# unilight/jatts

Hardware: AMD Instinct MI355X
Metric: audio samples/sec (22.05 kHz) + RTF, FastSpeech2+HiFi-GAN (higher is better)
Workload: dtype f32 (emulated: 3 exact bf16 terms per operand, 7 MFMA products, f32 accumulate; attention / norms / duration predictor exact f32); 1 GPU; FastSpeech2(JSUT conformer 4+4, adim 384)+HiFi-GAN v1 22k, 64 utts x 128 phonemes x 6 frames per GPU; hop=256, parallelism=dp1 (utterance sharding, int16 PCM all-gather)

## Files before the change

### include/jatts_hip.h

```cpp
#ifndef JATTS_HIP_H_
#define JATTS_HIP_H_

#include <stdint.h>

#ifdef __cplusplus
extern "C" {
#endif

#define JATTS_ABI_VERSION 7

#define JATTS_F32 0
#define JATTS_F16 1
#define JATTS_F32S 2
#define JATTS_F32E 3
#define JATTS_F32E6 4

#define JATTS_ACT_NONE 0
#define JATTS_ACT_RELU 1
#define JATTS_ACT_TANH 2
#define JATTS_ACT_SWISH 3
#define JATTS_ACT_MISH 4
#define JATTS_ACT_SNAKEBETA 5

#define JATTS_PAD_ZERO 0
// ... 64 lines not shown
int jatts_conv1d(const jatts_conv_desc* d, void* stream);

int64_t jatts_conv_weight_index(int32_t n, int32_t tap, int32_t c, int32_t n_pad, int32_t c_in);

typedef struct jatts_resunit_desc {
  jatts_ragged rg;
  int32_t dtype;
  int32_t channels;
  int32_t k_w;
  int32_t dil;
  float slope;
  const void* x;
  void* y;
  const void* w1;
  const float* b1;
  const void* w2;
  const float* b2;
  const void* add0;
  const void* add1;
  float out_scale;
  const float* ws1;
  const float* ws2;
  int32_t w_layout;
  int32_t variant;
} jatts_resunit_desc;

int jatts_hifigan_resunit(const jatts_resunit_desc* d, void* stream);

int jatts_resunit_variant(const jatts_resunit_desc* d);

int jatts_resunit_single_conv(int32_t dtype, int32_t w_layout);

int64_t jatts_unit_weight_index_k32(int32_t n, int32_t tap, int32_t c, int32_t channels);

typedef struct jatts_resblock_desc {
  jatts_ragged rg;
  int32_t dtype;
  int32_t channels;
  int32_t k_w;
  int32_t n_units;
  int32_t dil[3];
  float slope;
  const void* x;
  void* y;
  const void* w1[3];
  const float* b1[3];
  const void* w2[3];
  const float* b2[3];
  const void* add0;
  const void* add1;
  float out_scale;
  const float* ws1[3];
  const float* ws2[3];
} jatts_resblock_desc;

int jatts_hifigan_resblock(const jatts_resblock_desc* d, void* stream);

int jatts_masked_loss(const jatts_ragged* rg, const float* a, int32_t lda, const float* b, int32_t ldb, int32_t dim,
                      const int32_t* valid_len, int32_t kind, float log_offset, double scale, float* out, double* workspace,
                      void* stream);
int jatts_conv1d_wgrad(const jatts_ragged* rg, const float* x, int32_t ldx, const float* dy, int32_t ldy, int32_t c_in,
                       int32_t n_out, int32_t k_w, int32_t dil, int32_t pad, float* dw, float* db, float* workspace, void* stream);
int jatts_pack_conv_weight(const float* w, int32_t n_out, int32_t c_in, int32_t k_w, int32_t c_mult, int32_t mode, int32_t dtype,
                           void* out, void* stream);
int jatts_pack_conv_weight_split(const float* w, int32_t n_out, int32_t c_in, int32_t k_w, int32_t c_mult, int32_t mode, void* out, float* inv,
                                 void* stream);
int jatts_pack_conv_weight_bf16x3(const float* w, int32_t n_out, int32_t c_in, int32_t k_w, int32_t c_mult, int32_t dgrad, void* out, void* stream);
int jatts_conv1d_wgrad_emul(const jatts_ragged* rg, const float* x, int32_t ldx, const float* dy, int32_t ldy, int32_t c_in, int32_t n_out, int32_t k_w,
                            int32_t dil, int32_t pad, int32_t dtype, float* dw, float* db, float* workspace, void* stream);
int jatts_col_sum(const float* x, int32_t ld, int64_t rows, int32_t dim, float* out, void* stream);

int jatts_layernorm_bwd(const float* x, int32_t ldx, const float* dy, int32_t lddy, const float* gamma, int64_t rows, int32_t dim,
                        float eps, float* dx, int32_t lddx, float* dgamma, float* dbeta, void* stream);
int jatts_act_fwd(int32_t mode, const float* x, float* y, int64_t n, void* stream);
int jatts_act_bwd(int32_t mode, const float* x, const float* dy, float* dx, int64_t n, void* stream);
int jatts_glu_fwd(const float* x, float* y, int64_t rows, int32_t dim, void* stream);
int jatts_glu_bwd(const float* x, const float* dy, float* dx, int64_t rows, int32_t dim, void* stream);
int jatts_dwconv(const jatts_ragged* rg, const float* x, const float* w, const float* bias, float* y, int32_t dim, int32_t k_w,
                 int32_t pad, int32_t flip, void* stream);
int jatts_dwconv_wgrad(const jatts_ragged* rg, const float* x, const float* dy, float* dw, int32_t dim, int32_t k_w, int32_t pad,
                       void* stream);
int jatts_col_stats(const float* x, const float* y2, int32_t ld, int64_t rows, int32_t dim, const float* shift, const float* mul,
                    int32_t mode, float* out0, float* out1, void* stream);
int jatts_bn_bwd_apply(const float* x, const float* dy, int64_t rows, int32_t dim, const float* mean, const float* rstd,
                       const float* gamma, const float* s_dy, const float* s_dyx, float* dx, void* stream);
int jatts_index_add_rows(const float* src, int32_t ld, const int64_t* idx, int64_t rows, int32_t dim, float scale, int64_t skip,
                         int64_t n_dst, float* dst, void* stream);
int jatts_lr_segment_sum(const jatts_ragged* rg, const int64_t* cum, const int32_t* cu_out, const float* dy, int32_t dim, float* dhs,
                         void* stream);
int jatts_shift_softmax_fwd(const float* ac, const float* bd, int32_t n_batch, int32_t n_heads, int32_t t_len, const int32_t* lens,
                            float scale, int32_t shift_mode, float* p, void* stream);
int jatts_shift_softmax_bwd(const float* p, const float* dp, int32_t n_batch, int32_t n_heads, int32_t t_len, float scale,
                            int32_t shift_mode, float* ds, float* dbd, void* stream);
int jatts_gate_bwd(const float* x, const float* dy, float* dx, int64_t rows, int32_t dim, void* stream);
int jatts_weight_norm_fwd(const float* v, const float* g, int32_t n_out, int32_t row_len, float* w, float* inv_norm, void* stream);
int jatts_weight_norm_bwd(const float* v, const float* g, const float* inv_norm, const float* dw, int32_t n_out, int32_t row_len,
                          float* dv, float* dg, void* stream);
int jatts_split_add(const float* o, const float* h, const float* skip, int64_t rows, int32_t dim, float* h_out, float* skip_out, void* stream);
int jatts_concat2(const float* a, const float* b, int64_t rows, int32_t dim, float* out, void* stream);
int jatts_outer_rows(const float* v, const float* w, const float* bias, int64_t rows, int32_t dim, int32_t accumulate, float* out,
                     void* stream);
int jatts_col_wsum(const float* x, int32_t ld, const float* v, int64_t rows, int32_t dim, float* out, void* stream);
int jatts_row_dot(const float* x, int32_t ld, const float* w, const float* bias, int64_t rows, int32_t dim, float* y, void* stream);
int jatts_masked_loss_bwd(const jatts_ragged* rg, const float* a, int32_t lda, const float* b, int32_t ldb, int32_t dim,
                          const int32_t* valid_len, int32_t kind, float log_offset, float scale, const float* upstream, float* da,
                          int32_t ldda, void* stream);
// ... 221 lines not shown
```

### jatts_amd/_abi.py

```python
import ctypes as C
import os

_HERE = os.path.dirname(os.path.abspath(__file__))
LIB_PATH = os.environ.get("JATTS_HIP_LIB") or os.path.join(_HERE, "lib", "libjatts_hip.so")

F32, F16, F32S, F32E, F32E6 = 0, 1, 2, 3, 4
ABI_VERSION = 7
ACT_NONE, ACT_RELU, ACT_TANH, ACT_SWISH, ACT_MISH, ACT_SNAKEBETA = 0, 1, 2, 3, 4, 5
PRE_NONE, PRE_LRELU = 0, 1
PAD_ZERO, PAD_REFLECT = 0, 1
STATS_ROWS_PER_GROUP = 1024


class Ragged(C.Structure):
    _fields_ = [("cu_rows", C.c_void_p), ("n_seq", C.c_int32), ("max_len", C.c_int32),
                ("len_mul", C.c_int32), ("total_rows", C.c_int32), ("host_lens", C.c_void_p)]


class ConvDesc(C.Structure):
    _fields_ = [
        ("rg", Ragged), ("dtype", C.c_int32), ("n_in", C.c_int32), ("x", C.c_void_p * 3),
        ("ldx", C.c_int32), ("in_scale", C.c_float), ("pre_act", C.c_int32), ("pre_slope", C.c_float),
        ("w", C.c_void_p), ("c_in", C.c_int32), ("n_out", C.c_int32), ("k_w", C.c_int32),
        ("dil", C.c_int32), ("pad", C.c_int32), ("bias", C.c_void_p), ("act", C.c_int32),
        ("alpha", C.c_float), ("resid", C.c_void_p), ("ldr", C.c_int32), ("y", C.c_void_p),
        ("ldy", C.c_int32), ("y_is_f32", C.c_int32), ("y_transposed", C.c_int32), ("y_seq_col0", C.c_void_p),
        ("pad_mode", C.c_int32), ("variant", C.c_int32), ("w_inv", C.c_void_p), ("act_a", C.c_void_p), ("act_b", C.c_void_p),
        ("n_split", C.c_int32), ("ldy2", C.c_int32), ("y2", C.c_void_p), ("y2_seq_col0", C.c_void_p), ("w_layout", C.c_int32),
        ("tap_group_n", C.c_int32), ("tap_a0", C.c_int32), ("tap_b0", C.c_int32), ("tap_k", C.c_int32),
    ]


class ResUnitDesc(C.Structure):
    _fields_ = [
        ("rg", Ragged), ("dtype", C.c_int32), ("channels", C.c_int32), ("k_w", C.c_int32),
        ("dil", C.c_int32), ("slope", C.c_float), ("x", C.c_void_p), ("y", C.c_void_p),
        ("w1", C.c_void_p), ("b1", C.c_void_p), ("w2", C.c_void_p), ("b2", C.c_void_p),
        ("add0", C.c_void_p), ("add1", C.c_void_p), ("out_scale", C.c_float),
        ("ws1", C.c_void_p), ("ws2", C.c_void_p), ("w_layout", C.c_int32), ("variant", C.c_int32),
    ]


class ResBlockDesc(C.Structure):
    _fields_ = [
        ("rg", Ragged), ("dtype", C.c_int32), ("channels", C.c_int32), ("k_w", C.c_int32), ("n_units", C.c_int32),
        ("dil", C.c_int32 * 3), ("slope", C.c_float), ("x", C.c_void_p), ("y", C.c_void_p),
        ("w1", C.c_void_p * 3), ("b1", C.c_void_p * 3), ("w2", C.c_void_p * 3), ("b2", C.c_void_p * 3),
        ("add0", C.c_void_p), ("add1", C.c_void_p), ("out_scale", C.c_float),
        ("ws1", C.c_void_p * 3), ("ws2", C.c_void_p * 3),
    ]


class RelAttnDesc(C.Structure):
    _fields_ = [
        ("rg", Ragged), ("dtype", C.c_int32), ("n_heads", C.c_int32), ("d_k", C.c_int32),
        ("q", C.c_void_p), ("ldq", C.c_int32), ("k", C.c_void_p), ("ldk", C.c_int32),
        ("vt", C.c_void_p), ("ldvt", C.c_int32), ("g", C.c_void_p), ("ldg", C.c_int32),
        ("ku", C.c_void_p), ("scale", C.c_float), ("out", C.c_void_p), ("ldo", C.c_int32),
        ("rel_mode", C.c_int32), ("rel_center", C.c_int32), ("vt_col0", C.c_void_p), ("kv_len", C.c_void_p),
    ]


COLLATE_MAX_FIELDS = 8


class CollateField(C.Structure):
    _fields_ = [("src", C.c_void_p), ("row_start", C.c_void_p), ("row_len", C.c_void_p), ("dst", C.c_void_p),
                ("elem_bytes", C.c_int32), ("dim", C.c_int32), ("t_max", C.c_int32)]


PROTOTYPES = {
    "jatts_abi_version": (C.c_int, []),
    "jatts_last_error": (C.c_char_p, []),
    "jatts_device_info": (C.c_int, [C.c_char_p, C.c_int]),
    "jatts_conv1d": (C.c_int, [C.POINTER(ConvDesc), C.c_void_p]),
    "jatts_conv_weight_index": (C.c_int64, [C.c_int32] * 5),
    "jatts_hifigan_resunit": (C.c_int, [C.POINTER(ResUnitDesc), C.c_void_p]),
    "jatts_resunit_variant": (C.c_int, [C.POINTER(ResUnitDesc)]),
    "jatts_resunit_single_conv": (C.c_int, [C.c_int32, C.c_int32]),
    "jatts_unit_weight_index_k32": (C.c_int64, [C.c_int32] * 4),
    "jatts_hifigan_resblock": (C.c_int, [C.POINTER(ResBlockDesc), C.c_void_p]),
    "jatts_debug_trace": (C.c_int, [C.c_void_p, C.c_int64]),
    "jatts_mfma_probe": (C.c_int, [C.c_int32, C.c_int32, C.c_void_p, C.c_int64, C.c_int32, C.c_int32, C.c_void_p, C.c_void_p, C.c_void_p]),
    "jatts_mfma_probe_flops": (C.c_double, [C.c_int32, C.c_int32, C.c_int32]),
    "jatts_set_workspace": (C.c_int, [C.c_void_p, C.c_int64]),
    "jatts_pack_conv_weight_split": (C.c_int, [C.c_void_p, C.c_int32, C.c_int32, C.c_int32, C.c_int32, C.c_int32, C.c_void_p, C.c_void_p, C.c_void_p]),
    "jatts_bgemm": (C.c_int, [C.c_void_p, C.c_int64, C.c_int64, C.c_int32, C.c_int32, C.c_void_p, C.c_int64, C.c_int64, C.c_int32, C.c_int32,
                              C.c_void_p, C.c_int64, C.c_int64, C.c_int32, C.c_int32, C.c_int32, C.c_int32, C.c_int32, C.c_int32, C.c_float,
                              C.c_int32, C.c_void_p]),
    "jatts_bgemm_emul": (C.c_int, [C.c_void_p, C.c_int64, C.c_int64, C.c_int32, C.c_int32, C.c_void_p, C.c_int64, C.c_int64, C.c_int32, C.c_int32,
                                   C.c_void_p, C.c_int64, C.c_int64, C.c_int32, C.c_int32, C.c_int32, C.c_int32, C.c_int32, C.c_int32, C.c_float,
                                   C.c_int32, C.c_int32, C.c_void_p]),
    "jatts_pcm16": (C.c_int, [C.c_void_p, C.c_int64, C.c_void_p, C.c_void_p]),
    "jatts_alignment_logp": (C.c_int, [C.POINTER(Ragged), C.c_void_p, C.c_int32, C.c_void_p, C.c_void_p, C.c_int32,
                                       C.c_void_p, C.c_int32, C.c_void_p]),
    "jatts_alignment_logp_bwd": (C.c_int, [C.POINTER(Ragged), C.c_void_p, C.c_int32, C.c_void_p, C.c_void_p, C.c_int32, C.c_void_p, C.c_int32,
                                           C.c_void_p, C.c_int32, C.c_void_p, C.c_void_p, C.c_void_p, C.c_void_p]),
    "jatts_mas_viterbi": (C.c_int, [C.POINTER(Ragged), C.c_void_p, C.c_void_p, C.c_int32, C.c_int32, C.c_void_p,
                                    C.c_void_p, C.c_void_p, C.c_void_p]),
    "jatts_hifigan_output": (C.c_int, [C.POINTER(Ragged), C.c_int32, C.POINTER(C.c_void_p), C.c_int32,
                                       C.c_float, C.c_float, C.c_int32, C.c_int32, C.c_void_p, C.c_float,
                                       C.c_void_p, C.c_void_p]),
# ... 161 lines not shown
```

### jatts_amd/csrc/conv_api.hip

```cpp
#include <stdlib.h>

#include "common.h"

unsigned long long* jatts_g_trace = nullptr;
unsigned jatts_g_trace_cap = 0;

int jatts_conv1d_f16(const jatts_conv_desc& d, hipStream_t s);
int jatts_conv1d_f32(const jatts_conv_desc& d, hipStream_t s);
int jatts_conv1d_split(const jatts_conv_desc& d, hipStream_t s);
int jatts_conv1d_emul(const jatts_conv_desc& d, hipStream_t s);
int jatts_resunit_f16_narrow(const jatts_resunit_desc& d, hipStream_t s);
int jatts_resunit_f16_wide(const jatts_resunit_desc& d, hipStream_t s);
int jatts_resunit_f32(const jatts_resunit_desc& d, hipStream_t s);
int jatts_resunit_split(const jatts_resunit_desc& d, hipStream_t s);
int jatts_resunit_emul(const jatts_resunit_desc& d, hipStream_t s, int* pick);
int jatts_resunit1_f16(const jatts_resunit_desc& d, hipStream_t s);
int jatts_resunit1_f32(const jatts_resunit_desc& d, hipStream_t s);
int jatts_resunit1_emul(const jatts_resunit_desc& d, hipStream_t s);
int jatts_resblock_f16(const jatts_resblock_desc& d, hipStream_t s);
int jatts_resblock_f32(const jatts_resblock_desc& d, hipStream_t s);
int jatts_resblock_split(const jatts_resblock_desc& d, hipStream_t s);
int jatts_resblock_emul(const jatts_resblock_desc& d, hipStream_t s);

extern "C" int jatts_debug_trace(void* buf, int64_t n_workgroups) {
// ... 80 lines not shown
  if (d->dtype != JATTS_F16 && d->dtype != JATTS_F32) return jatts_set_error_msg(JATTS_ERR_UNSUPPORTED, "resunit: unsupported channels/dtype (use jatts_conv1d)");
  return JATTS_OK;
}

extern "C" int jatts_hifigan_resunit(const jatts_resunit_desc* d, void* stream) {
  if (const int rc = resunit_check(d)) return rc;
  hipStream_t s = (hipStream_t)stream;
  if (!d->w2) {
    if (const int rc = resunit1_check(d)) return rc;
    if (d->rg.max_len <= 0) return JATTS_OK;
    if (d->dtype == JATTS_F16) return jatts_resunit1_f16(*d, s);
    if (d->dtype == JATTS_F32) return jatts_resunit1_f32(*d, s);
    return jatts_resunit1_emul(*d, s);
  }
  if (d->rg.max_len <= 0) return JATTS_OK;
  if (d->dtype == JATTS_F16) return d->channels <= 64 ? jatts_resunit_f16_narrow(*d, s) : jatts_resunit_f16_wide(*d, s);
  if (d->dtype == JATTS_F32) return jatts_resunit_f32(*d, s);
  if (d->dtype == JATTS_F32S) {
    if (!d->ws1 || !d->ws2) return jatts_set_error_msg(JATTS_ERR_ARG, "resunit: JATTS_F32S needs ws1 / ws2");
    return jatts_resunit_split(*d, s);
  }
  if (d->dtype == JATTS_F32E || d->dtype == JATTS_F32E6) {
    if (d->w_layout != 0 && d->w_layout != 1) return jatts_set_error_msg(JATTS_ERR_ARG, "resunit: w_layout must be 0 or 1");
    return jatts_resunit_emul(*d, s, nullptr);
  }
  if (d->w_layout != 0) return jatts_set_error_msg(JATTS_ERR_ARG, "resunit: w_layout = 1 goes with JATTS_F32E / JATTS_F32E6 only");
  return jatts_set_error_msg(JATTS_ERR_UNSUPPORTED, "resunit: unsupported channels/dtype (use jatts_conv1d)");
}

extern "C" int jatts_resunit_variant(const jatts_resunit_desc* d) {
  if (const int rc = resunit_check(d)) return rc;
  int form = 1;
  if (!d->w2) {
    const int rc = resunit1_check(d);
    return rc ? rc : 1;
  }
  if (d->rg.max_len > 0 && (d->dtype == JATTS_F32E || d->dtype == JATTS_F32E6)) {
    if (d->w_layout != 0 && d->w_layout != 1) return jatts_set_error_msg(JATTS_ERR_ARG, "resunit: w_layout must be 0 or 1");
    if (const int rc = jatts_resunit_emul(*d, nullptr, &form)) return rc;
  }
  return form;
}

extern "C" int jatts_hifigan_resblock(const jatts_resblock_desc* d, void* stream) {
  if (!d || !d->x || !d->y || !d->rg.cu_rows) return jatts_set_error_msg(JATTS_ERR_ARG, "resblock: null pointer");
  if (d->n_units < 1 || d->n_units > 3) return jatts_set_error_msg(JATTS_ERR_ARG, "resblock: 1..3 units");
  for (int u = 0; u < d->n_units; ++u) {
    if (!d->w1[u] || !d->w2[u] || !d->b1[u] || !d->b2[u]) return jatts_set_error_msg(JATTS_ERR_ARG, "resblock: null weights");
    if (d->dil[u] < 1) return jatts_set_error_msg(JATTS_ERR_ARG, "resblock: dil >= 1 required");
  }
  if (d->x == d->y) return jatts_set_error_msg(JATTS_ERR_ARG, "resblock: y must not alias x");
  if (d->k_w < 1 || !(d->k_w & 1)) return jatts_set_error_msg(JATTS_ERR_ARG, "resblock: odd k_w required");
  if (!(d->slope >= 0.f && d->slope <= 1.f)) return jatts_set_error_msg(JATTS_ERR_ARG, "resblock: LeakyReLU slope must be in [0, 1]");
  if (d->dtype == JATTS_F32S) {
    for (int u = 0; u < d->n_units; ++u)
      if (!d->ws1[u] || !d->ws2[u]) return jatts_set_error_msg(JATTS_ERR_ARG, "resblock: JATTS_F32S needs ws1 / ws2");
    if (d->rg.max_len <= 0) return JATTS_OK;
    return jatts_resblock_split(*d, (hipStream_t)stream);
  }
  if (d->dtype == JATTS_F32E || d->dtype == JATTS_F32E6) {
    if (d->rg.max_len <= 0) return JATTS_OK;
    return jatts_resblock_emul(*d, (hipStream_t)stream);
  }
  if (d->dtype != JATTS_F16 && d->dtype != JATTS_F32) return jatts_set_error_msg(JATTS_ERR_ARG, "resblock: unknown dtype");
  if (d->rg.max_len <= 0) return JATTS_OK;
  return d->dtype == JATTS_F16 ? jatts_resblock_f16(*d, (hipStream_t)stream) : jatts_resblock_f32(*d, (hipStream_t)stream);
}
```

### jatts_amd/csrc/resblock_emul.hip

```cpp
#include "resblock_emul_impl.h"

template <typename T>
static int resblock_emul(const jatts_resblock_desc& d, hipStream_t s) {
  switch (d.channels) {
    case 32:
      return launch_resblock_emul<T, 32, 256, 1, 2, 2, 2>(d, s);
    case 64:
      return launch_resblock_emul<T, 64, 128, 2, 2, 2, 2>(d, s);
  }
  return jatts_set_error_msg(JATTS_ERR_UNSUPPORTED, "resblock (emulated): 32 / 64 channels only (use jatts_hifigan_resunit)");
}

int jatts_resblock_emul(const jatts_resblock_desc& d, hipStream_t s) { return d.dtype == JATTS_F32E6 ? resblock_emul<bf3f>(d, s) : resblock_emul<bf3>(d, s); }
```

### jatts_amd/csrc/resunit_emul16_impl.h

```cpp
#pragma once
#include <type_traits>

#include "resunit_emul_impl.h"

#ifndef JATTS_U16_ROWS
#define JATTS_U16_ROWS 1
#endif
#ifndef JATTS_U16_DIAG
#define JATTS_U16_DIAG 0
#endif

namespace {

struct acc2x4 { f32x4 big, small; };
template <typename T> struct Acc16 { typedef f32x4 type; };
template <> struct Acc16<bf3p<7>> { typedef acc2x4 type; };
__device__ __forceinline__ void acc16_set(f32x4& a, int i, float v) { a[i] = v; }
__device__ __forceinline__ void acc16_set(acc2x4& a, int i, float v) { a.small[i] = v; a.big[i] = 0.f; }
__device__ __forceinline__ void acc16_finish(f32x4&) {}
__device__ __forceinline__ void acc16_finish(acc2x4& a) { a.small = a.big + a.small; }
__device__ __forceinline__ f32x4& acc16_val(f32x4& a) { return a; }
__device__ __forceinline__ f32x4& acc16_val(acc2x4& a) { return a.small; }

template <int P> __device__ __forceinline__ void mma16p(const bf3px8<7>& a, const bf3px8<7>& b, acc2x4& c) {
// ... 357 lines not shown
        for (int e = 0; e < 4; ++e) {
          const float a = acc16_val(acc[f][t])[e] * keep;
          v[e] = fmaxf(a, a * d.slope);
        }
        bf16x4 q0, q1, q2;
        bf3_split4(v, q0, q1, q2);
        char* p = hs + (size_t)(col + off) * pitch + (size_t)(n0 >> 3) * 48 + (size_t)(n0 & 4) * 2;
        *reinterpret_cast<bf16x4*>(p) = q0;
        *reinterpret_cast<bf16x4*>(p + 16) = q1;
        *reinterpret_cast<bf16x4*>(p + 32) = q2;
      }
    }
    JATTS_STAMP(12);
    lds_barrier();
    JATTS_STAMP(4);

    bias_acc(bs + C);
    ws.bind((const T*)d.w2, KC32, NFR16, nf0, lane);
    conv16<T, NF, NT, KC32>(acc, ws, 0, K, 1, hs, pitch, col0, lane, nullptr);
    finish_acc();
    JATTS_STAMP(5);

    __syncthreads();
    if constexpr (SLIDE) {
      for (int u = tid; u < (K - 1) * (C / 8); u += NTHR) {
        const int r = u / (C / 8), cu = u % (C / 8);
        Vec8IO<T>::sts(tl + (size_t)r * pitch_t + (size_t)cu * 48, Vec8IO<T>::lds(hs + (size_t)(nout + r) * pitch + (size_t)cu * 48));
      }
    }
    char* ys = smem;
#pragma unroll
    for (int t = 0; t < NT; ++t) {
      const int col = col0 + t * 16 + (lane & 15);
      if (col >= nvalid) continue;
#pragma unroll
      for (int f = 0; f < NF; ++f) {
        const int n0 = (nf0 + f) * 16 + 4 * g4;
        *reinterpret_cast<f32x4*>(ys + (size_t)col * pitch + (size_t)n0 * 4) = acc16_val(acc[f][t]);
      }
    }
    __syncthreads();
    JATTS_STAMP(6);
    {
      const int vrows = nvalid;
      const int64_t g0 = (seq_row0 + t0) * (int64_t)C;
      constexpr bool keep_small = C <= 64;
      const float* xg = (const float*)d.x;
      float* yg = (float*)d.y;
      if constexpr (RREG) {
        constexpr int UPR = C / 8;
        const int n_out = vrows * UPR;
        const bool has_add1 = d.add0 != nullptr && d.add1 != nullptr;
        f32x8 a0[MAXI], a1[MAXI];
        if (d.add0) {
#pragma unroll
          for (int j = 0; j < MAXI; ++j) {
            const int v = tid + j * NTHR;
            if (v < n_out) {
              a0[j] = Vec8IO<float>::ldg((const float*)d.add0 + g0 + (int64_t)v * 8);
              if (has_add1) a1[j] = Vec8IO<float>::ldg((const float*)d.add1 + g0 + (int64_t)v * 8);
            }
          }
        }
#pragma unroll
        for (int j = 0; j < MAXI; ++j) {
          const int v = tid + j * NTHR;
          if (v >= n_out) continue;
          const int ro = v / UPR, cu = v - ro * UPR;
          f32x8 o = Vec8IO<float>::lds(ys + (size_t)ro * pitch + (size_t)cu * 32);
#pragma unroll
          for (int e = 0; e < 8; ++e) o[e] = o[e] + xk[j][e];
          if (d.add0) {
#pragma unroll
            for (int e = 0; e < 8; ++e) o[e] = (o[e] + a0[j][e] + (has_add1 ? a1[j][e] : 0.f)) * d.out_scale;
          }
          float* dst = yg + g0 + (int64_t)v * 8;
          *reinterpret_cast<f32x4*>(dst) = f32x4{o[0], o[1], o[2], o[3]};
          *reinterpret_cast<f32x4*>(dst + 4) = f32x4{o[4], o[5], o[6], o[7]};
        }
      } else {
        if (d.add0) unit_store_pass<float, C, keep_small ? 2 : 4, true, NTHR>(d.add0, d.add1, d.out_scale, ys, pitch, vrows, xg, yg, g0);
        else unit_store_pass<float, C, keep_small ? 4 : 8, false, NTHR>(d.add0, d.add1, d.out_scale, ys, pitch, vrows, xg, yg, g0);
      }
    }
    JATTS_STAMP(7);
    if constexpr (!SLIDE) break;
    t0 += nout;
    slide = true;
    if (t0 >= L) {
      f_seq += L;
      if (f_seq >= f_end) break;
      do { ++b; } while (d.rg.cu_rows[b + 1] == d.rg.cu_rows[b]);
      t0 = 0;
      slide = false;
    } else if (f_seq + t0 >= f_end) {
      break;
    }
  }
  JATTS_TRACE_END();
}

inline int resunit16_pick(const jatts_resunit_desc& d, int runs, int wgcols, bool slide_auto, bool slide_fits) {
  const int64_t positions = ragged_is_1d(d.rg) ? (int64_t)d.rg.total_rows * d.rg.len_mul : (int64_t)d.rg.n_seq * d.rg.max_len * d.rg.len_mul;
  const bool slide = d.variant == 2 || (d.variant == 0 && slide_auto && positions >= 2 * (int64_t)runs * wgcols);
  return slide && slide_fits ? 2 : 1;
}

template <typename T, int C, int WGCOLS, int WN, int WT, int OCC = 2, bool KSPLIT = false, bool RREG = false>
int launch_resunit_emul16(const jatts_resunit_desc& d, hipStream_t s, int* pick) {
  const int K = d.k_w, p2 = (K - 1) / 2, p1 = p2 * d.dil;
  const int tt_out = WGCOLS - 2 * p2;
  if (tt_out < 8) return jatts_set_error_msg(JATTS_ERR_UNSUPPORTED, "resunit: kernel too wide for tile");
  const size_t pitch = C * 6 + 16, pitch_x = KSPLIT ? (C / 2) * 6 + 16 : pitch;
  const size_t rows_x = WGCOLS + 2 * p1, rows_h = WGCOLS + K - 1;
  if (KSPLIT && 2 * p1 > 64) return jatts_set_error_msg(JATTS_ERR_UNSUPPORTED, "resunit (emulated, channel halves): halo beyond 32 rows a side");
  const size_t region = rows_x * pitch_x > rows_h * pitch ? rows_x * pitch_x : rows_h * pitch;
  const size_t tail = (size_t)(K - 1) * C * 6;
  const size_t lds = region + 2 * C * sizeof(float);
  if (lds > 160 * 1024) return jatts_set_error_msg(JATTS_ERR_UNSUPPORTED, "resunit: tile exceeds 160 KiB LDS");
  int dev = 0, cus = 0;
  hipError_t e = hipGetDevice(&dev);
  if (e == hipSuccess) e = hipDeviceGetAttribute(&cus, hipDeviceAttributeMultiprocessorCount, dev);
  if (e != hipSuccess) return jatts_set_error(e, __FILE__, __LINE__);
  const int runs = cus * OCC;
  const int form = resunit16_pick(d, runs, WGCOLS, !RREG, lds + tail <= 160 * 1024);
  if (pick) {
    *pick = form;
    return JATTS_OK;
  }
  if (form == 2) {
    constexpr auto kern = resunit_emul16_kernel<T, C, WGCOLS, WN, WT, OCC, KSPLIT, RREG, true>;
    if (const int rc = unit_lds_ready<kern>(JATTS_SITE("resunit: tile exceeds 160 KiB LDS"), lds + tail)) return rc;
    hipLaunchKernelGGL(kern, dim3((unsigned)runs), dim3(WN * WT * 64), lds + tail, s, d, jatts_g_trace, jatts_g_trace_cap, (unsigned)(region + tail));
    JATTS_CHECK_LAUNCH();
    return JATTS_OK;
  }
  constexpr auto kern = resunit_emul16_kernel<T, C, WGCOLS, WN, WT, OCC, KSPLIT, RREG>;
  return unit_launch<kern>(JATTS_SITE("resunit: tile exceeds 160 KiB LDS"), WN * WT * 64, lds, tt_out, d.rg, s, d, jatts_g_trace, jatts_g_trace_cap, (unsigned)region);
}

}
```

### jatts_amd/hip.py

```python
import collections
import contextlib
import ctypes as C

import torch

from . import _abi
from . import precision as _precision
from ._abi import ACT_MISH, ACT_NONE, ACT_RELU, ACT_SWISH, ACT_TANH, F16, F32, F32E, F32E6, F32S
from .precision import EMUL, PRECISIONS

_TORCH = {F32: torch.float32, F16: torch.float16, F32S: torch.float32, F32E: torch.float32, F32E6: torch.float32}


def torch_dtype(code):
    return _TORCH[code]


def code_of(t):
    if t.dtype == torch.float32:
        return F32
    if t.dtype == torch.float16:
        return F16
    raise TypeError(f"unsupported dtype {t.dtype}")

# ... 620 lines not shown


def _check_unit_weights(who, dtype, channels, k_w, *ws):
    n = channels * channels * k_w
    want = {F32: (torch.float32, n), F16: (torch.float16, n), F32S: (torch.float16, 2 * n), F32E: (torch.bfloat16, 3 * n), F32E6: (torch.bfloat16, 3 * n)}[dtype]
    for w in ws:
        if w.dtype != want[0] or w.numel() != want[1] or not w.is_cuda:
            raise ValueError(f"{who}: dtype code {dtype} needs packed weights of {want[1]} x {want[0]} on the GPU (pack_conv_weight / pack_conv_weight_split / "
                             f"pack_conv_weight_bf16x3 with c_mult=32), got {w.numel()} x {w.dtype}")


def _resunit_desc(rb, len_mul, x, y, w1, b1, w2, b2, channels, k_w, dil, slope, dtype, add, out_scale, ws, w_layout, variant):
    d = _abi.ResUnitDesc()
    d.w_layout, d.variant = w_layout, variant
    d.rg = rb.struct(len_mul)
    d.dtype, d.channels, d.k_w, d.dil, d.slope = dtype, channels, k_w, dil, slope
    rows = rb.total * len_mul
    if x.numel() != rows * channels or y.numel() != rows * channels or x.dtype != torch_dtype(dtype):
        raise ValueError("hifigan_resunit: bad buffer size/dtype")
    d.x, d.y = _dev(x).data_ptr(), y.data_ptr()
    _check_unit_weights("hifigan_resunit", dtype, channels, k_w, *((w1,) if w2 is None else (w1, w2)))
    d.w1, d.b1, d.w2, d.b2 = w1.data_ptr(), b1.data_ptr(), _ptr(w2), _ptr(b2)
    if dtype == F32S:
        need = ws[:1] if ws is not None and w2 is None else ws
        if need is None or any(v is None or v.numel() < channels or v.dtype != torch.float32 for v in need):
            raise ValueError("hifigan_resunit: F32S needs the inverse weight scales (pack_conv_weight_split)")
        d.ws1, d.ws2 = ws[0].data_ptr(), _ptr(ws[1]) if len(ws) > 1 else None
    if add:
        for a in add:
            if a.numel() != rows * channels or a.dtype != x.dtype:
                raise ValueError("hifigan_resunit: bad mix buffer")
        d.add0 = add[0].data_ptr()
        d.add1 = add[1].data_ptr() if len(add) > 1 else None
    d.out_scale = out_scale
    return d


def hifigan_resunit(rb, len_mul, x, y, w1, b1, w2, b2, channels, k_w, dil, slope, dtype, add=None, out_scale=1.0, ws=None, w_layout=0, variant=0):
    lib = _abi.load()
    d = _resunit_desc(rb, len_mul, x, y, w1, b1, w2, b2, channels, k_w, dil, slope, dtype, add, out_scale, ws, w_layout, variant)
    with _Timed("resunit", (channels, k_w, dil, rb.total * len_mul, len(add) if add else 0)):
        _abi.check(lib.jatts_hifigan_resunit(C.byref(d), _stream()), "jatts_hifigan_resunit")
    return y


def resunit_variant(rb, len_mul, x, y, w1, b1, w2, b2, channels, k_w, dil, slope, dtype, add=None, out_scale=1.0, ws=None, w_layout=0, variant=0):
    lib = _abi.load()
    d = _resunit_desc(rb, len_mul, x, y, w1, b1, w2, b2, channels, k_w, dil, slope, dtype, add, out_scale, ws, w_layout, variant)
    rc = lib.jatts_resunit_variant(C.byref(d))
    _abi.check(min(rc, 0), "jatts_resunit_variant")
    return rc


def hifigan_resblock(rb, len_mul, x, y, units, channels, k_w, slope, dtype, add=None, out_scale=1.0, ws=None):
    lib = _abi.load()
    d = _abi.ResBlockDesc()
    d.rg = rb.struct(len_mul)
    d.dtype, d.channels, d.k_w, d.n_units, d.slope = dtype, channels, k_w, len(units), slope
    rows = rb.total * len_mul
    if x.numel() != rows * channels or y.numel() != rows * channels or x.dtype != torch_dtype(dtype):
        raise ValueError("hifigan_resblock: bad buffer size/dtype")
    d.x, d.y = _dev(x).data_ptr(), y.data_ptr()
    for i, (w1, b1, w2, b2, dil) in enumerate(units):
        _check_unit_weights("hifigan_resblock", dtype, channels, k_w, w1, w2)
        d.w1[i], d.b1[i], d.w2[i], d.b2[i], d.dil[i] = w1.data_ptr(), b1.data_ptr(), w2.data_ptr(), b2.data_ptr(), dil
    if dtype == F32S:
        if ws is None or len(ws) != len(units):
            raise ValueError("hifigan_resblock: F32S needs the inverse weight scales of every unit")
        for i, (a, b) in enumerate(ws):
            d.ws1[i], d.ws2[i] = a.data_ptr(), b.data_ptr()
    if add:
        for a in add:
            if a.numel() != rows * channels or a.dtype != x.dtype:
                raise ValueError("hifigan_resblock: bad mix buffer")
        d.add0 = add[0].data_ptr()
        d.add1 = add[1].data_ptr() if len(add) > 1 else None
    d.out_scale = out_scale
    with _Timed("resblock", (channels, k_w, tuple(u[4] for u in units), rows, len(add) if add else 0)):
        _abi.check(lib.jatts_hifigan_resblock(C.byref(d), _stream()), "jatts_hifigan_resblock")
    return y


def hifigan_output(rb, len_mul, xs, in_scale, slope, c_in, k_w, w, bias, dtype):
    lib = _abi.load()
    rows = rb.total * len_mul
    y = torch.empty(rows, dtype=torch.float32, device=xs[0].device)
    arr = (C.c_void_p * len(xs))(*[_dev(x).data_ptr() for x in xs])
    rg = rb.struct(len_mul)
    _abi.check(lib.jatts_hifigan_output(C.byref(rg), dtype, arr, len(xs), in_scale, slope, c_in, k_w,
                                        w.data_ptr(), float(bias), y.data_ptr(), _stream()),
               "jatts_hifigan_output")
    return y


def relpos_attention(rb, q, ldq, k, ldk, vt, ldvt, g, ldg, ku, scale, n_heads, d_k, dtype,
                     q_col0=0, k_col0=0, rel_mode=1, rel_center=0, vt_col0=None, kv_len=None):
    lib = _abi.load()
    out = torch.empty(rb.total, n_heads * d_k, dtype=torch_dtype(dtype), device=q.device)
    d = _abi.RelAttnDesc()
    d.rg = rb.struct()
    d.dtype, d.n_heads, d.d_k = dtype, n_heads, d_k
    d.q, d.ldq = _ptr(_dev(q), q_col0), ldq
    d.k, d.ldk = _ptr(k, k_col0), ldk
    d.vt, d.ldvt = vt.data_ptr(), ldvt
    d.g, d.ldg = _ptr(g), ldg
    d.ku = _ptr(ku)
    d.scale = scale
    d.out, d.ldo = out.data_ptr(), n_heads * d_k
    d.rel_mode, d.rel_center = rel_mode, rel_center
# ... 1336 lines not shown
```

### jatts_amd/vocoder/hifigan.py

```python

import torch

from .. import hip
from ..graphs import GraphCache
from ..hip import PackedConv
from ..models._prepared import Prepared
from ..models import _schema as S
from ..precision import TABLE


class UnitConv:

    def __init__(self, w, b, code, k32=False, also32=False):
        self.n_out, self.c_in, self.k = w.shape
        self.inv, self.layout = None, 1 if (k32 and code in hip.EMUL) else 0
        if code == hip.F32S:
            self.w, self.inv = hip.pack_conv_weight_split(w, 32)
        elif code in hip.EMUL:
            self.w = hip.pack_unit_weight_bf16x3_k32(w) if k32 else hip.pack_conv_weight_bf16x3(w, 32)
        else:
            self.w = hip.pack_conv_weight(w, code, 32)
        self.w_block = hip.pack_conv_weight_bf16x3(w, 32) if (self.layout and also32) else self.w
        self.b = b.detach().float().contiguous()


class HiFiGANGenerator(Prepared, torch.nn.Module):
    def __init__(self, in_channels=80, out_channels=1, channels=512, kernel_size=7,
                 upsample_scales=(8, 8, 2, 2), upsample_kernel_sizes=(16, 16, 4, 4),
                 resblock_kernel_sizes=(3, 7, 11), resblock_dilations=((1, 3, 5), (1, 3, 5), (1, 3, 5)),
                 use_additional_convs=True, bias=True, nonlinear_activation="LeakyReLU",
                 nonlinear_activation_params=None, use_weight_norm=True, **unused):
        super().__init__()
        if nonlinear_activation != "LeakyReLU":
            raise NotImplementedError("only LeakyReLU generators are supported")
        if out_channels != 1:
            raise NotImplementedError("out_channels must be 1")
        self.use_additional_convs, self.bias = bool(use_additional_convs), bool(bias)
        if len(upsample_scales) != len(upsample_kernel_sizes):
            raise ValueError("upsample_scales / upsample_kernel_sizes mismatch")
        self.slope = float((nonlinear_activation_params or {"negative_slope": 0.1}).get("negative_slope", 0.1))
        self.in_channels, self.channels, self.kernel_size = in_channels, channels, kernel_size
        self.upsample_scales = tuple(int(s) for s in upsample_scales)
        self.upsample_kernel_sizes = tuple(int(k) for k in upsample_kernel_sizes)
        self.resblock_kernel_sizes = tuple(int(k) for k in resblock_kernel_sizes)
        self.resblock_dilations = tuple(tuple(int(d) for d in ds) for ds in resblock_dilations)
        if channels % (1 << len(self.upsample_scales)) or channels > 512:
            raise NotImplementedError("channels must be divisible by 2**n_upsamples and <= 512")
        for s_, uk in zip(self.upsample_scales, self.upsample_kernel_sizes):
            if uk != 2 * s_:
                raise NotImplementedError(f"upsample_kernel_size {uk} != 2 * scale {s_}: only the k = 2s geometry of the HiFi-GAN recipes is supported")
        if not 1 <= len(self.resblock_kernel_sizes) <= 3:
            raise NotImplementedError("1..3 ResBlocks per stage (the MRF mix kernels take up to 3 inputs)")
        self.hop = 1
        for s in self.upsample_scales:
            self.hop *= s
        spec = S.new_spec()
        S._conv(spec, "input_conv", channels, in_channels, kernel_size)
        nb = len(self.resblock_kernel_sizes)
        c = channels
        for i, uk in enumerate(self.upsample_kernel_sizes):
            spec[f"upsamples.{i}.1.weight"] = ((c, c // 2, uk), "param")
            if self.bias:
                spec[f"upsamples.{i}.1.bias"] = ((c // 2,), "param")
            c //= 2
            for j, rk in enumerate(self.resblock_kernel_sizes):
                for d in range(len(self.resblock_dilations[j])):
                    S._conv(spec, f"blocks.{i * nb + j}.convs1.{d}.1", c, c, rk, bias=self.bias)
                    if self.use_additional_convs:
                        S._conv(spec, f"blocks.{i * nb + j}.convs2.{d}.1", c, c, rk, bias=self.bias)
        S._conv(spec, "output_conv.1", out_channels, c, kernel_size)
        S.build_from_spec(self, spec)
        self.eval()

    def load_state_dict(self, state_dict, strict=True, **kw):
        sd = {}
# ... 26 lines not shown

    def _prepare_packed(self, dev, key, dt):
        udt = TABLE[self.precision].operand
        sd = self.state_dict()
        f32 = lambda t: t.detach().float().to(dev).contiguous()
        fset, fhalo = {hip.F16: (self.fused_blocks, 64), hip.F32: (self.fused_blocks_f32, 16), hip.F32S: (self.fused_blocks_split, 64)}.get(
            udt, (self.fused_blocks_emul, 64))
        P = {"key": key, "dtype": dt, "dev": dev, "unit_dtype": udt, "fused_blocks": fset, "fused_halo": fhalo}
        nb = len(self.resblock_kernel_sizes)
        P["ups"], P["blocks"] = [], []
        supported = {hip.F16: (32, 64, 128, 256, 512), hip.F32: (32, 64, 128, 256)}[dt]
        P["unit_channels"] = supported

        def cp(c):
            for v in supported:
                if c <= v:
                    return v
            raise NotImplementedError(f"{c} channels exceed the widest fused-unit tile for this precision")

        def padw(w, n, c):
            w = w.detach().float()
            o = torch.zeros(n, c, w.shape[2], dtype=torch.float32)
            o[: w.shape[0], : w.shape[1]] = w
            return o

        def padb(b, n):
            o = torch.zeros(n, dtype=torch.float32)
            if b is not None:
                o[: b.numel()] = b.detach().float()
            return o

        c_prev = hip.round_up(self.channels, 64)
        P["in"] = PackedConv(padw(sd["input_conv.weight"], c_prev, sd["input_conv.weight"].shape[1]), padb(sd["input_conv.bias"], c_prev), dt, dev)
        for i, (s, uk) in enumerate(zip(self.upsample_scales, self.upsample_kernel_sizes)):
            w = sd[f"upsamples.{i}.1.weight"].detach().float()
            c_out = cp(w.shape[1])
            if i + 1 < len(self.upsample_scales):
                c_out = max(c_out, 64)
            wp = torch.zeros(c_prev, c_out, w.shape[2], dtype=torch.float32)
            wp[: w.shape[0], : w.shape[1]] = w
            wc, pad = hip.convtranspose_as_conv(wp, s, s // 2 + s % 2)
            tg = hip.convtranspose_tap_groups(uk, s, s // 2 + s % 2)
            win = None if tg is None else (tg[0] * c_out,) + tg[1:]
            if win is not None:
                hip.check_tap_window(wc, win)
            pc = PackedConv(wc, padb(sd.get(f"upsamples.{i}.1.bias"), c_out).repeat(s), dt, dev)
            P["ups"].append((pc, pad, s, c_out, win))
            stage = []
            for j, rk in enumerate(self.resblock_kernel_sizes):
                units = []
                for di, d in enumerate(self.resblock_dilations[j]):
                    q = f"blocks.{i * nb + j}."
                    k32 = c_out % 32 == 0
                    also32 = self.use_additional_convs and (c_out, rk) in self.fused_blocks_emul
                    mk = lambda w, b: UnitConv(w, b, udt, k32, also32)
                    c1 = mk(padw(sd[q + f"convs1.{di}.1.weight"], c_out, c_out).to(dev), padb(sd.get(q + f"convs1.{di}.1.bias"), c_out).to(dev))
                    c2 = mk(padw(sd[q + f"convs2.{di}.1.weight"], c_out, c_out).to(dev), padb(sd.get(q + f"convs2.{di}.1.bias"), c_out).to(dev)) \
                        if self.use_additional_convs else None
                    units.append((c1, c2, rk, d))
                stage.append(units)
            P["blocks"].append(stage)
            c_prev = c_out
        wo = padw(sd["output_conv.1.weight"], 1, c_prev)
        P["out_w"] = f32(wo[0].t())
        P["out_b"] = float(sd["output_conv.1.bias"].detach().float()[0])
        self._prep = P
        return P

    fused_blocks = frozenset({(32, 3), (32, 7), (64, 3)})
    fused_blocks_f32 = frozenset({(32, 3)})
    fused_blocks_split = frozenset({(32, 3), (32, 7), (64, 3)})

    fused_blocks_emul = frozenset({(32, 3)})

    @torch.no_grad()
    def inference_batch(self, rb, mel, scale=None, shift=None, taps=None):
        P = self._prepare()
        if rb.n_seq == 1 and taps is None:
            gc = P.get("graphs")
            if gc is None:
                gc = P["graphs"] = GraphCache()
            affine = tuple(t for t in (scale, shift) if t is not None)

            def body(mel_, *aff):
                it = iter(aff)
                return self._generate(P, hip.RaggedBatch(rb.lens, rb.device), mel_, next(it) if scale is not None else None,
                                      next(it) if shift is not None else None, None)
            return gc.run(("generate", rb.total, scale is not None, shift is not None), body, (mel,) + affine)
        return self._generate(P, rb, mel, scale, shift, taps)

    def _generate(self, P, rb, mel, scale, shift, taps):
        dt, udt = P["dtype"], P["unit_dtype"]
        pin = P["in"]
        x = hip.affine_cast(mel, dt, scale=scale, shift=shift, ldy=pin.c_in)
        x = pin(rb, x)
        if taps is not None:
            taps["input_conv"] = x.float()
        xs, in_scale, rate = [x], 1.0, 1
        supported = P["unit_channels"]
        for i, (pc, pad, s, c_out, win) in enumerate(P["ups"]):
            rows = rb.total * rate
            up = pc(rb, xs, pad=pad, pre_lrelu=self.slope, in_scale=in_scale, len_mul=rate, tap_window=win)
            rate *= s
            up = up.view(rows * s, c_out)
            if taps is not None:
                taps[f"up{i}"] = up.float()
            outs = []
            blocks = P["blocks"][i]
            fuse_mean = c_out in supported and len(blocks) in (2, 3)
            bufs = [[torch.empty_like(up), torch.empty_like(up)] for _ in blocks]
            for j, units in enumerate(blocks):
                cur = up
                if self.use_additional_convs and (c_out, units[0][2]) in P["fused_blocks"] and len(units) <= 3 \
                        and sum((units[0][2] - 1) // 2 * (u[3] + 1) for u in units) <= P["fused_halo"]:
                    lastb = fuse_mean and j == len(blocks) - 1
                    hip.hifigan_resblock(rb, rate, cur, bufs[j][0], [(c1.w_block, c1.b, c2.w_block, c2.b, d) for c1, c2, _, d in units],
                                         c_out, units[0][2], self.slope, udt, add=outs if lastb else None,
                                         out_scale=1.0 / len(blocks) if lastb else 1.0,
                                         ws=[(c1.inv, c2.inv) for c1, c2, _, _ in units] if udt == hip.F32S else None)
                    outs.append(bufs[j][0])
                    continue
                for di, (c1, c2, rk, d) in enumerate(units):
                    nxt = bufs[j][di & 1]
                    last = fuse_mean and j == len(blocks) - 1 and di == len(units) - 1
                    hip.hifigan_resunit(rb, rate, cur, nxt, c1.w, c1.b, c2.w if c2 else None, c2.b if c2 else None, c_out, rk, d, self.slope, udt,
                                        add=outs if last else None, out_scale=1.0 / len(blocks) if last else 1.0,
                                        ws=(c1.inv, c2.inv) if udt == hip.F32S else None, w_layout=c1.layout)
                    cur = nxt
                outs.append(cur)
            if fuse_mean:
                xs, in_scale = [outs[-1]], 1.0
            else:
                xs, in_scale = outs, 1.0 / len(outs)
            if taps is not None:
                taps[f"mrf{i}"] = sum(o.float() for o in xs) * in_scale
        return hip.hifigan_output(rb, rate, xs, in_scale, 0.01, xs[0].shape[1], self.kernel_size,
                                  P["out_w"], P["out_b"], dt)

    @torch.no_grad()
    def inference(self, c, normalize_before=False):
        if normalize_before:
            raise NotImplementedError("normalize_before=True needs registered stats; jatts passes False (vocoder.py:64)")
        if not isinstance(c, torch.Tensor):
            c = torch.tensor(c, dtype=torch.float)
        dev = self.input_conv.weight.device
        c = c.to(dev).float().contiguous()
        rb = hip.RaggedBatch([c.shape[0]], dev)
        return self.inference_batch(rb, c).view(-1, 1)
```

Baseline: 70.22 million samples/s.

## Add k32-layout fused emulated resblock kernel and size-gated sliding resunit variant

Adds a new fused HiFi-GAN resblock kernel for the bf16x3-emulated path that consumes the k32 (layout 1) packed weights directly. The old path packed a second copy of the weights in the older layout just for the fused block. The new kernel streams weights through WStream16/conv16, keeps residuals in registers and runs all units in one launch over an LDS tile. It also adds a resunit variant 3 that enables the sliding kernel by problem size for (64, 11) units, and zero-initialises the add buffers in the sliding store. This removes the duplicate weight packing and lets the fused block use the faster 16-wide MFMA weight layout, with possible register-pressure and occupancy risk.

```diff
diff --git a/include/jatts_hip.h b/include/jatts_hip.h
--- a/include/jatts_hip.h
+++ b/include/jatts_hip.h
@@ -140,6 +140,7 @@
   float out_scale;
   const float* ws1[3];
   const float* ws2[3];
+  int32_t w_layout;
 } jatts_resblock_desc;
 
 int jatts_hifigan_resblock(const jatts_resblock_desc* d, void* stream);
diff --git a/jatts_amd/_abi.py b/jatts_amd/_abi.py
--- a/jatts_amd/_abi.py
+++ b/jatts_amd/_abi.py
@@ -47,7 +47,7 @@
         ("dil", C.c_int32 * 3), ("slope", C.c_float), ("x", C.c_void_p), ("y", C.c_void_p),
         ("w1", C.c_void_p * 3), ("b1", C.c_void_p * 3), ("w2", C.c_void_p * 3), ("b2", C.c_void_p * 3),
         ("add0", C.c_void_p), ("add1", C.c_void_p), ("out_scale", C.c_float),
-        ("ws1", C.c_void_p * 3), ("ws2", C.c_void_p * 3),
+        ("ws1", C.c_void_p * 3), ("ws2", C.c_void_p * 3), ("w_layout", C.c_int32),
     ]
 
 
diff --git a/jatts_amd/csrc/conv_api.hip b/jatts_amd/csrc/conv_api.hip
--- a/jatts_amd/csrc/conv_api.hip
+++ b/jatts_amd/csrc/conv_api.hip
@@ -156,6 +156,8 @@
   if (d->x == d->y) return jatts_set_error_msg(JATTS_ERR_ARG, "resblock: y must not alias x");
   if (d->k_w < 1 || !(d->k_w & 1)) return jatts_set_error_msg(JATTS_ERR_ARG, "resblock: odd k_w required");
   if (!(d->slope >= 0.f && d->slope <= 1.f)) return jatts_set_error_msg(JATTS_ERR_ARG, "resblock: LeakyReLU slope must be in [0, 1]");
+  if (d->w_layout != 0 && d->dtype != JATTS_F32E && d->dtype != JATTS_F32E6)
+    return jatts_set_error_msg(JATTS_ERR_ARG, "resblock: w_layout = 1 goes with JATTS_F32E / JATTS_F32E6 only");
   if (d->dtype == JATTS_F32S) {
     for (int u = 0; u < d->n_units; ++u)
       if (!d->ws1[u] || !d->ws2[u]) return jatts_set_error_msg(JATTS_ERR_ARG, "resblock: JATTS_F32S needs ws1 / ws2");
@@ -163,6 +165,7 @@
     return jatts_resblock_split(*d, (hipStream_t)stream);
   }
   if (d->dtype == JATTS_F32E || d->dtype == JATTS_F32E6) {
+    if (d->w_layout != 0 && d->w_layout != 1) return jatts_set_error_msg(JATTS_ERR_ARG, "resblock: w_layout must be 0 or 1");
     if (d->rg.max_len <= 0) return JATTS_OK;
     return jatts_resblock_emul(*d, (hipStream_t)stream);
   }
diff --git a/jatts_amd/csrc/resblock_emul.hip b/jatts_amd/csrc/resblock_emul.hip
--- a/jatts_amd/csrc/resblock_emul.hip
+++ b/jatts_amd/csrc/resblock_emul.hip
@@ -1,4 +1,9 @@
 #include "resblock_emul_impl.h"
+#include "resblock_emul16_impl.h"
+
+#ifndef JATTS_RB16_C64_WIDE
+#define JATTS_RB16_C64_WIDE 0
+#endif
 
 template <typename T>
 static int resblock_emul(const jatts_resblock_desc& d, hipStream_t s) {
@@ -11,4 +16,22 @@
   return jatts_set_error_msg(JATTS_ERR_UNSUPPORTED, "resblock (emulated): 32 / 64 channels only (use jatts_hifigan_resunit)");
 }
 
-int jatts_resblock_emul(const jatts_resblock_desc& d, hipStream_t s) { return d.dtype == JATTS_F32E6 ? resblock_emul<bf3f>(d, s) : resblock_emul<bf3>(d, s); }
+template <typename T>
+static int resblock_emul16(const jatts_resblock_desc& d, hipStream_t s) {
+  switch (d.channels) {
+    case 32:
+      return launch_resblock_emul16<T, 32, 256, 1, 4, 2>(d, s);
+    case 64:
+#if JATTS_RB16_C64_WIDE
+      return launch_resblock_emul16<T, 64, 256, 1, 4, 1>(d, s);
+#else
+      return launch_resblock_emul16<T, 64, 128, 2, 2, 2>(d, s);
+#endif
+  }
+  return jatts_set_error_msg(JATTS_ERR_UNSUPPORTED, "resblock (emulated): 32 / 64 channels only (use jatts_hifigan_resunit)");
+}
+
+int jatts_resblock_emul(const jatts_resblock_desc& d, hipStream_t s) {
+  if (d.w_layout == 1) return d.dtype == JATTS_F32E6 ? resblock_emul16<bf3f>(d, s) : resblock_emul16<bf3>(d, s);
+  return d.dtype == JATTS_F32E6 ? resblock_emul<bf3f>(d, s) : resblock_emul<bf3>(d, s);
+}
diff --git a/jatts_amd/csrc/resblock_emul16_impl.h b/jatts_amd/csrc/resblock_emul16_impl.h
--- /dev/null
+++ b/jatts_amd/csrc/resblock_emul16_impl.h
@@ -0,0 +1,217 @@
+#pragma once
+#include "resunit_emul16_impl.h"
+
+namespace {
+
+template <typename T, int C, int WGCOLS, int WN, int WT, int OCC>
+__global__ __launch_bounds__(WN* WT * 64, OCC) void resblock_emul16_kernel(jatts_resblock_desc d, unsigned bias_off) {
+  typedef typename Elem<T>::vec8 V8;
+  extern __shared__ __attribute__((aligned(16))) char smem[];
+  constexpr int NF = C / (WN * 16), NT = WGCOLS / (WT * 16);
+  constexpr int KC32 = C / 32, NFR16 = C / 16;
+  constexpr int pitch = C * 6 + 16;
+  constexpr int NTHR = WN * WT * 64;
+  constexpr int UPR = C / 8;
+  static_assert(NF * WN * 16 == C && NT * WT * 16 == WGCOLS && C % 32 == 0, "tile shape");
+  static_assert(sizeof(T) == 6, "bf3 is three packed bf16");
+
+  const int K = d.k_w, p2 = (K - 1) / 2, NU = d.n_units;
+  int H = 0, M = 0;
+  for (int u = 0; u < NU; ++u) {
+    H += p2 * (d.dil[u] + 1);
+    M = max(M, p2 * d.dil[u]);
+  }
+  const int tt_out = WGCOLS - 2 * H;
+  unit_window win;
+  if (!unit_window_of(d.rg, tt_out, win)) return;
+  const int L = win.L, t0 = win.t0;
+  const int64_t seq_row0 = win.seq_row0;
+  const int lane = threadIdx.x & 63, wave = threadIdx.x >> 6;
+  const int wn = wave / WT, wt = wave % WT;
+  const int g4 = lane >> 4;
+  const int col0 = wt * NT * 16;
+  const int nf0 = wn * NF;
+  const int rows = WGCOLS + 2 * M;
+
+  float* bs = reinterpret_cast<float*>(smem + bias_off);
+  for (int u = threadIdx.x; u < 2 * C * NU; u += NTHR) {
+    const int un = u / (2 * C), r = u - un * 2 * C;
+    bs[u] = r < C ? d.b1[un][r] : d.b2[un][r - C];
+  }
+
+  WStream16<T, NF> ws;
+  ws.bind((const T*)d.w1[0], KC32, NFR16, nf0, lane);
+  ws.fetch(0, 0);
+  const float* xg = (const float*)d.x;
+  constexpr int MAXU = ((WGCOLS + 64) * UPR + NTHR - 1) / NTHR;
+  f32x8 xv[MAXU];
+  {
+    const int total = rows * UPR, pos0 = t0 - H - M;
+#pragma unroll
+    for (int j = 0; j < MAXU; ++j) {
+      const int u = threadIdx.x + j * NTHR;
+      const int r = u / UPR, cu = u - r * UPR;
+      const int pos = pos0 + r;
+      if (u < total && pos >= 0 && pos < L) xv[j] = Vec8IO<float>::ldg(xg + (seq_row0 + pos) * (int64_t)C + cu * 8);
+      else xv[j] = f32x8{0, 0, 0, 0, 0, 0, 0, 0};
+    }
+#pragma unroll
+    for (int j = 0; j < MAXU; ++j) {
+      const int u = threadIdx.x + j * NTHR;
+      if (u < total) Vec8IO<float>::sts(smem + (size_t)(u / UPR) * pitch + (size_t)(u % UPR) * 32, xv[j]);
+    }
+  }
+  __syncthreads();
+  f32x4 resid[NF][NT];
+  bool keep[NT];
+#pragma unroll
+  for (int t = 0; t < NT; ++t) {
+    const int col = col0 + t * 16 + (lane & 15);
+    const int pos = t0 - H + col;
+    keep[t] = pos >= 0 && pos < L;
+#pragma unroll
+    for (int f = 0; f < NF; ++f)
+      resid[f][t] = *reinterpret_cast<const f32x4*>(smem + (size_t)(M + col) * pitch + (size_t)((nf0 + f) * 16 + 4 * g4) * 4);
+  }
+  __syncthreads();
+  {
+    const int total = rows * UPR;
+#pragma unroll
+    for (int j = 0; j < MAXU; ++j) {
+      const int u = threadIdx.x + j * NTHR;
+      if (u >= total) continue;
+      lrelu8(xv[j], d.slope);
+      V8 o;
+      bf3_split8(xv[j], o);
+      Vec8IO<T>::sts(smem + (size_t)(u / UPR) * pitch + (size_t)(u % UPR) * 48, o);
+    }
+  }
+  __syncthreads();
+
+  typename Acc16<T>::type acc[NF][NT];
+  auto put_planes = [&]() {
+#pragma unroll
+    for (int t = 0; t < NT; ++t) {
+      const int col = col0 + t * 16 + (lane & 15);
+#pragma unroll
+      for (int f = 0; f < NF; ++f) {
+        const int n0 = (nf0 + f) * 16 + 4 * g4;
+        float v[4];
+#pragma unroll
+        for (int e = 0; e < 4; ++e) v[e] = acc16_val(acc[f][t])[e];
+        bf16x4 q0, q1, q2;
+        bf3_split4(v, q0, q1, q2);
+        char* p = smem + (size_t)(M + col) * pitch + (size_t)(n0 >> 3) * 48 + (size_t)(n0 & 4) * 2;
+        *reinterpret_cast<bf16x4*>(p) = q0;
+        *reinterpret_cast<bf16x4*>(p + 16) = q1;
+        *reinterpret_cast<bf16x4*>(p + 32) = q2;
+      }
+    }
+  };
+  auto bias_acc = [&](const float* bv) {
+#pragma unroll
+    for (int f = 0; f < NF; ++f) {
+      const f32x4 bb = *reinterpret_cast<const f32x4*>(bv + (nf0 + f) * 16 + 4 * g4);
+#pragma unroll
+      for (int t = 0; t < NT; ++t)
+#pragma unroll
+        for (int e = 0; e < 4; ++e) acc16_set(acc[f][t], e, bb[e]);
+    }
+  };
+  auto finish_acc = [&]() {
+#pragma unroll
+    for (int f = 0; f < NF; ++f)
+#pragma unroll
+      for (int t = 0; t < NT; ++t) acc16_finish(acc[f][t]);
+  };
+  auto first_step = [&](const void* w) { return (const T*)w + (size_t)nf0 * 512 + (size_t)lane * 8; };
+
+  int hv = 0;
+  auto col_ok = [&](int t) {
+    const int col = col0 + t * 16 + (lane & 15);
+    return keep[t] && col >= hv && col < WGCOLS - hv;
+  };
+  for (int u = 0; u < NU; ++u) {
+    const int dil = d.dil[u], p1 = p2 * dil;
+    const float* bu = bs + (size_t)u * 2 * C;
+    if (u > 0) hv += p1;
+    bias_acc(bu);
+    ws.bind((const T*)d.w1[u], KC32, NFR16, nf0, lane);
+    conv16<T, NF, NT, KC32>(acc, ws, 0, K, dil, smem + (size_t)(M - p1) * pitch, pitch, col0, lane, first_step(d.w2[u]));
+    finish_acc();
+#pragma unroll
+    for (int t = 0; t < NT; ++t) {
+      const bool ok = col_ok(t);
+#pragma unroll
+      for (int f = 0; f < NF; ++f)
+#pragma unroll
+        for (int e = 0; e < 4; ++e) {
+          const float a = ok ? acc16_val(acc[f][t])[e] : 0.f;
+          acc16_val(acc[f][t])[e] = fmaxf(a, a * d.slope);
+        }
+    }
+    lds_barrier();
+    put_planes();
+    hv += p2;
+    lds_barrier();
+    const bool last = u == NU - 1;
+    bias_acc(bu + C);
+    ws.bind((const T*)d.w2[u], KC32, NFR16, nf0, lane);
+    conv16<T, NF, NT, KC32>(acc, ws, 0, K, 1, smem + (size_t)(M - p2) * pitch, pitch, col0, lane, last ? nullptr : first_step(d.w1[last ? u : u + 1]));
+    finish_acc();
+#pragma unroll
+    for (int t = 0; t < NT; ++t) {
+      const bool ok = col_ok(t);
+#pragma unroll
+      for (int f = 0; f < NF; ++f) {
+        f32x4 xn;
+#pragma unroll
+        for (int e = 0; e < 4; ++e) {
+          xn[e] = ok ? acc16_val(acc[f][t])[e] + resid[f][t][e] : 0.f;
+          acc16_val(acc[f][t])[e] = last ? xn[e] : fmaxf(xn[e], xn[e] * d.slope);
+        }
+        resid[f][t] = xn;
+      }
+    }
+    lds_barrier();
+    if (!last) put_planes();
+    else {
+#pragma unroll
+      for (int t = 0; t < NT; ++t) {
+        const int col = col0 + t * 16 + (lane & 15);
+#pragma unroll
+        for (int f = 0; f < NF; ++f)
+          *reinterpret_cast<f32x4*>(smem + (size_t)(M + col) * pitch + (size_t)((nf0 + f) * 16 + 4 * g4) * 4) = acc16_val(acc[f][t]);
+      }
+    }
+    lds_barrier();
+  }
+
+  {
+    const int vrows = min(tt_out, L - t0);
+    const int64_t g0 = (seq_row0 + t0) * (int64_t)C;
+    const char* ys = smem + (size_t)(M + H) * pitch;
+    unit_store<float, C, NTHR, false>(d, ys, pitch, vrows, g0);
+  }
+}
+
+template <typename T, int C, int WGCOLS, int WN, int WT, int OCC>
+int launch_resblock_emul16(const jatts_resblock_desc& d, hipStream_t s) {
+  const int p2 = (d.k_w - 1) / 2;
+  int H = 0, M = 0;
+  for (int u = 0; u < d.n_units; ++u) {
+    H += p2 * (d.dil[u] + 1);
+    M = M > p2 * d.dil[u] ? M : p2 * d.dil[u];
+  }
+  const int tt_out = WGCOLS - 2 * H;
+  if (tt_out < 32) return jatts_set_error_msg(JATTS_ERR_UNSUPPORTED, "resblock (emulated): receptive field too wide for the tile");
+  if (2 * M > 64) return jatts_set_error_msg(JATTS_ERR_UNSUPPORTED, "resblock (emulated): margin beyond 32 rows a side");
+  const size_t pitch = C * 6 + 16;
+  size_t lds = (size_t)(WGCOLS + 2 * M) * pitch;
+  const unsigned bias_off = (unsigned)lds;
+  lds += (size_t)d.n_units * 2 * C * sizeof(float);
+  constexpr auto kern = resblock_emul16_kernel<T, C, WGCOLS, WN, WT, OCC>;
+  return unit_launch<kern>(JATTS_SITE("resblock (emulated): tile exceeds 160 KiB LDS"), WN * WT * 64, lds, tt_out, d.rg, s, d, bias_off);
+}
+
+}
diff --git a/jatts_amd/csrc/resunit_emul16_impl.h b/jatts_amd/csrc/resunit_emul16_impl.h
--- a/jatts_amd/csrc/resunit_emul16_impl.h
+++ b/jatts_amd/csrc/resunit_emul16_impl.h
@@ -433,6 +433,10 @@
         const int n_out = vrows * UPR;
         const bool has_add1 = d.add0 != nullptr && d.add1 != nullptr;
         f32x8 a0[MAXI], a1[MAXI];
+        if constexpr (SLIDE) {
+#pragma unroll
+          for (int j = 0; j < MAXI; ++j) a0[j] = a1[j] = f32x8{0, 0, 0, 0, 0, 0, 0, 0};
+        }
         if (d.add0) {
 #pragma unroll
           for (int j = 0; j < MAXI; ++j) {
@@ -483,7 +487,8 @@
 
 inline int resunit16_pick(const jatts_resunit_desc& d, int runs, int wgcols, bool slide_auto, bool slide_fits) {
   const int64_t positions = ragged_is_1d(d.rg) ? (int64_t)d.rg.total_rows * d.rg.len_mul : (int64_t)d.rg.n_seq * d.rg.max_len * d.rg.len_mul;
-  const bool slide = d.variant == 2 || (d.variant == 0 && slide_auto && positions >= 2 * (int64_t)runs * wgcols);
+  const bool by_size = d.variant == 3 || (d.variant == 0 && slide_auto);
+  const bool slide = d.variant == 2 || (by_size && positions >= 2 * (int64_t)runs * wgcols);
   return slide && slide_fits ? 2 : 1;
 }
 
diff --git a/jatts_amd/hip.py b/jatts_amd/hip.py
--- a/jatts_amd/hip.py
+++ b/jatts_amd/hip.py
@@ -696,9 +696,10 @@
     return rc
 
 
-def hifigan_resblock(rb, len_mul, x, y, units, channels, k_w, slope, dtype, add=None, out_scale=1.0, ws=None):
+def hifigan_resblock(rb, len_mul, x, y, units, channels, k_w, slope, dtype, add=None, out_scale=1.0, ws=None, w_layout=0):
     lib = _abi.load()
     d = _abi.ResBlockDesc()
+    d.w_layout = w_layout
     d.rg = rb.struct(len_mul)
     d.dtype, d.channels, d.k_w, d.n_units, d.slope = dtype, channels, k_w, len(units), slope
     rows = rb.total * len_mul
diff --git a/jatts_amd/vocoder/hifigan.py b/jatts_amd/vocoder/hifigan.py
--- a/jatts_amd/vocoder/hifigan.py
+++ b/jatts_amd/vocoder/hifigan.py
@@ -11,7 +11,7 @@
 
 class UnitConv:
 
-    def __init__(self, w, b, code, k32=False, also32=False):
+    def __init__(self, w, b, code, k32=False):
         self.n_out, self.c_in, self.k = w.shape
         self.inv, self.layout = None, 1 if (k32 and code in hip.EMUL) else 0
         if code == hip.F32S:
@@ -20,7 +20,7 @@
             self.w = hip.pack_unit_weight_bf16x3_k32(w) if k32 else hip.pack_conv_weight_bf16x3(w, 32)
         else:
             self.w = hip.pack_conv_weight(w, code, 32)
-        self.w_block = hip.pack_conv_weight_bf16x3(w, 32) if (self.layout and also32) else self.w
+        self.w_block = self.w
         self.b = b.detach().float().contiguous()
 
 
@@ -153,8 +153,7 @@
                 for di, d in enumerate(self.resblock_dilations[j]):
                     q = f"blocks.{i * nb + j}."
                     k32 = c_out % 32 == 0
-                    also32 = self.use_additional_convs and (c_out, rk) in self.fused_blocks_emul
-                    mk = lambda w, b: UnitConv(w, b, udt, k32, also32)
+                    mk = lambda w, b: UnitConv(w, b, udt, k32)
                     c1 = mk(padw(sd[q + f"convs1.{di}.1.weight"], c_out, c_out).to(dev), padb(sd.get(q + f"convs1.{di}.1.bias"), c_out).to(dev))
                     c2 = mk(padw(sd[q + f"convs2.{di}.1.weight"], c_out, c_out).to(dev), padb(sd.get(q + f"convs2.{di}.1.bias"), c_out).to(dev)) \
                         if self.use_additional_convs else None
@@ -173,6 +172,7 @@
     fused_blocks_split = frozenset({(32, 3), (32, 7), (64, 3)})
 
     fused_blocks_emul = frozenset({(32, 3)})
+    sliding_units_emul = frozenset({(64, 11)})
 
     @torch.no_grad()
     def inference_batch(self, rb, mel, scale=None, shift=None, taps=None):
@@ -218,7 +218,7 @@
                     hip.hifigan_resblock(rb, rate, cur, bufs[j][0], [(c1.w_block, c1.b, c2.w_block, c2.b, d) for c1, c2, _, d in units],
                                          c_out, units[0][2], self.slope, udt, add=outs if lastb else None,
                                          out_scale=1.0 / len(blocks) if lastb else 1.0,
-                                         ws=[(c1.inv, c2.inv) for c1, c2, _, _ in units] if udt == hip.F32S else None)
+                                         ws=[(c1.inv, c2.inv) for c1, c2, _, _ in units] if udt == hip.F32S else None, w_layout=units[0][0].layout)
                     outs.append(bufs[j][0])
                     continue
                 for di, (c1, c2, rk, d) in enumerate(units):
@@ -226,7 +226,8 @@
                     last = fuse_mean and j == len(blocks) - 1 and di == len(units) - 1
                     hip.hifigan_resunit(rb, rate, cur, nxt, c1.w, c1.b, c2.w if c2 else None, c2.b if c2 else None, c_out, rk, d, self.slope, udt,
                                         add=outs if last else None, out_scale=1.0 / len(blocks) if last else 1.0,
-                                        ws=(c1.inv, c2.inv) if udt == hip.F32S else None, w_layout=c1.layout)
+                                        ws=(c1.inv, c2.inv) if udt == hip.F32S else None, w_layout=c1.layout,
+                                        variant=3 if c1.layout and c2 and (c_out, rk) in self.sliding_units_emul else 0)
                     cur = nxt
                 outs.append(cur)
             if fuse_mean:
```

Result: no change. 70.47 million samples/s, median of 6 (+0.4%).
